# Mr-LvGJ/kubernetes-scheduler

Hardware: AMD Instinct MI355X
Metric: pod-node pair evals/sec (filter+score+select) at 100k×100k; bit-exact picks (higher is better)
Workload: dtype u32+f32+f64

## Files before the change

### kubernetes-scheduler_amd/csrc/yoda_kernels.hip

```cpp
#include <hip/hip_runtime.h>
#include <stdint.h>
#include <algorithm>
#include <type_traits>
#include <cstdlib>

#include "yoda_layout.h"
#include "yoda_launch.h"
#include "yoda_modeb.h"

#if !defined(YODA_AB_KNOBS) &&                                                         \
    (defined(YODA_ABL_K1_NOGEN) || defined(YODA_ABL_K1_NOHC) || defined(YODA_ABL_K1_NOPART) || \
     defined(YODA_ABL_K1_NOBS) || defined(YODA_ABL_K1_NOBM))
#error "YODA_ABL_* ablations give wrong results: build them with -DYODA_AB_KNOBS (tools/build_ab.sh)"
#endif

#pragma clang fp contract(off)

namespace yoda {

constexpr int64_t kI64Max = 0x7fffffffffffffffll;

static inline dim3 pod_grid(uint32_t n) { return dim3((n + kBlock - 1) / kBlock); }

template <Path P>
// ... 2272 lines not shown
          const double os = ts[k];
          const uint32_t oi = ti[k];
          ts[k] = gt ? cs : os;
          ti[k] = gt ? ci : oi;
          cs = gt ? os : cs;
          ci = gt ? oi : ci;
        }
      }
    } else {
      if (raw > best) {
        best = raw;
        idx = n;
        ties = 1;
      } else if (raw == best) {
        ++ties;
      }
      low = fmin(low, raw);
    }
  };
  if (ms.bs) {
    const BlockMask* bsw = ms.bs + (size_t)w * ms.bs_stride;
    for (uint32_t nb = n0; nb < n1; nb += kWave) {
      if (!blk_listed(ms.blk, ms.blk_stride, w, nb >> 6)) continue;
      const BlockMask bk = bsw[nb >> 6];
      uint64_t bits = bk.nz;
      while (bits) {
        const uint32_t j = (uint32_t)__builtin_ctzll(bits);
        bits &= bits - 1;
        const uint32_t n = nb + j;
        const uint64_t mj = ((bk.full >> j) & 1ull) ? live_mask : bmw[n];
        if ((mj >> lane) & 1ull) visit(n);
      }
    }
  } else {
    for (uint32_t g = n0; g < n1; g += 8) {
      const Group<uint64_t, 8> mk = load_group<uint64_t, 8>(
          reinterpret_cast<const unsigned char*>(bmw + g));
      if ((mk.v[0] | mk.v[1] | mk.v[2] | mk.v[3] | mk.v[4] | mk.v[5] | mk.v[6] | mk.v[7]) == 0)
        continue;
#pragma unroll
      for (int j = 0; j < 8; ++j) {
        const uint32_t n = g + (uint32_t)j;
        if (mk.v[j] == 0 || n >= n1) continue;
        if ((mk.v[j] >> lane) & 1ull) visit(n);
      }
    }
  }
  if (!live) return;
  if constexpr (OUT == OUT_TOPK) {
#pragma unroll
    for (int k = 0; k < TK; ++k) {
      const size_t o = ((size_t)chunk * TK + k) * n_pods + p;
      tk_s[o] = ts[k];
      tk_i[o] = ti[k];
    }
  } else {
    const size_t o = (size_t)chunk * n_pods + p;
    pbest[o] = best;
    pidx[o] = idx;
    pties[o] = ties;
    plow[o] = low;
  }
}

#ifndef YODA_K2_WAVES
#define YODA_K2_WAVES 5
#endif
template <int K, bool STATS, int TKO = 0, bool RK = false, bool MIX = true, bool Q32 = true>
__global__ __launch_bounds__(kBlock) __attribute__((amdgpu_waves_per_eu(K <= 8 ? (TKO == 0 ? YODA_K2_WAVES : (TKO <= 8 ? 4 : 3)) : 1))) void k2_block_n32(
    const unsigned char* __restrict__ nodes, const unsigned char* __restrict__ sum2,
    uint32_t n_nodes, uint32_t chunk_nodes, ScoreArgs args, uint32_t n_pods,
    const uint64_t* __restrict__ bm, uint32_t bm_stride, const BlockMask* __restrict__ bs,
    uint32_t bs_stride, const uint64_t* __restrict__ blk,
    uint32_t blk_stride, double* __restrict__ pbest,
    uint32_t* __restrict__ pidx, uint32_t* __restrict__ pties, double* __restrict__ plow,
    unsigned long long* __restrict__ stats, uint64_t* __restrict__ tk_keys, uint32_t ib) {
  constexpr uint32_t S2 = k2sum_stride(K), NS = n32_stride(K), MS = mix_stride(K);
  constexpr bool TOPK = TKO > 0;
  constexpr int TL = TOPK ? TKO : 1;
  constexpr uint32_t PSW = K + 2;
  constexpr uint32_t TAB = kWave * PSW;
  constexpr uint32_t kSets = 4, REC = 16;
  constexpr uint32_t TT = (TOPK && !RK) ? (TKO > 8 ? 3u : 2u) : 1u;
  constexpr uint32_t RECS = TAB, RCPS = TAB + kWave * REC, IDW = RCPS + 16 * (kSets + 1),
                     XTAB = IDW + kWave, LDSW = XTAB + (TT - 1) * TAB;
  auto row_base = [&](uint32_t q) -> uint32_t { return q == 0 ? 0u : XTAB + (q - 1u) * TAB; };
  __shared__ __attribute__((aligned(16))) uint32_t lds_all[kBlock / kWave][LDSW];
  const uint32_t lane = lane_id();
  uint32_t* lds = lds_all[threadIdx.x >> 6];
  const Tile tl = tile();
  const uint32_t pbk = args.pb_order ? args.pb_order[tl.pb] : tl.pb;
  const uint32_t p = pbk * kBlock + threadIdx.x;
  const uint32_t chunk = tl.chunk;
  const uint32_t n0 = chunk * chunk_nodes;
  const uint32_t n1 = min(n0 + chunk_nodes, n_nodes);
  const bool live = p < n_pods;
  const uint64_t live_mask = ballot(live);
  if (live_mask == 0) return;
  const bool trace = STATS && (stats[15] & 0xffull) == 1ull;
  const uint64_t t_start = STATS ? wall_clock64() : 0ull;
  const uint64_t* bmw = bm + (size_t)uniform_u32(p >> 6) * bm_stride;
  const BlockMask* bsw = bs ? bs + (size_t)uniform_u32(p >> 6) * bs_stride : nullptr;
  using RS = std::conditional_t<Q32, float, double>;
  ScorerN32<RS> sc;
  if (live) sc.load(args, p, n_pods);
  static_assert((kKbLevels & (kKbLevels - 1u)) == 0u && kKbLevels <= kWave, "one level per lane");
  uint32_t lev = 0u;
  if (args.levels != nullptr) lev = args.levels[lane & (kKbLevels - 1u)];
  const bool act = live && (args.cnt == nullptr || args.cnt[p] != 0u);
  const uint64_t act_mask = ballot(act);
  bool seed_le_g = false;
  if constexpr (!TOPK) {
    if (args.seed != nullptr && args.g.tab != nullptr) {
      bool le;
      if constexpr (Q32)
        le = sc.r_bw >= args.g.f_bw && sc.r_core >= args.g.f_core && sc.r_pow >= args.g.f_pow;
      else
        le = sc.r_bw >= args.g.r_bw && sc.r_core >= args.g.r_core && sc.r_pow >= args.g.r_pow;
      le = le && sc.r_free >= args.g.r_free && sc.r_tot >= args.g.r_tot;
      seed_le_g = (ballot(act && !le) == 0ull);
    }
  }
  auto rl_d = [&](double x, int l) {
    const uint64_t b = (uint64_t)__double_as_longlong(x);
    return __longlong_as_double((long long)((uint64_t)(uint32_t)__builtin_amdgcn_readlane(
        (int)(uint32_t)b, l) | ((uint64_t)(uint32_t)__builtin_amdgcn_readlane(
        (int)(uint32_t)(b >> 32), l) << 32)));
  };
  uint32_t set = 0, nsets = 0;
  bool has_set = false;
  uint64_t rem = act_mask;
  auto rl_s = [&](RS x, int l) -> RS {
    if constexpr (Q32) return __int_as_float(__builtin_amdgcn_readlane(__float_as_int(x), l));
    else return rl_d(x, l);
  };
  RS u_bw = 0, u_core = 0, u_pow = 0;
  double u_free = 0.0, u_tot = 0.0;
  for (; rem != 0ull && nsets < kSets; ++nsets) {
    const int l = __builtin_ctzll(rem);
    const RS b_bw = rl_s(sc.r_bw, l), b_core = rl_s(sc.r_core, l), b_pow = rl_s(sc.r_pow, l);
    const double b_free = rl_d(sc.r_free, l), b_tot = rl_d(sc.r_tot, l);
    const bool in = act && sc.r_bw == b_bw && sc.r_core == b_core && sc.r_pow == b_pow &&
                    sc.r_free == b_free && sc.r_tot == b_tot;
    const uint64_t in_b = ballot(in) & rem;
    if ((in_b >> lane) & 1ull) {
      set = nsets;
      has_set = true;
    }
    rem &= ~in_b;
    if (nsets == 0) {
      u_bw = b_bw;
      u_core = b_core;
      u_pow = b_pow;
      u_free = b_free;
      u_tot = b_tot;
    }
    if (lane == (uint32_t)l) {
      RS* r = reinterpret_cast<RS*>(lds + RCPS + 16 * nsets);
      r[0] = b_bw;
      r[1] = b_core;
      r[2] = b_pow;
      double* d = reinterpret_cast<double*>(lds + RCPS + 16 * nsets + 8);
      d[0] = b_free;
      d[1] = b_tot;
    }
  }
  const bool uni_max = nsets <= 1u && rem == 0ull;
  const bool rec_ok = rem == 0ull;
  RS g_bw, g_core, g_pow;
  if constexpr (Q32) {
    g_bw = args.g.f_bw;
    g_core = args.g.f_core;
    g_pow = args.g.f_pow;
  } else {
    g_bw = args.g.r_bw;
    g_core = args.g.r_core;
    g_pow = args.g.r_pow;
  }
  const bool use_g = uni_max && args.g.tab != nullptr && u_bw == g_bw && u_core == g_core &&
                     u_pow == g_pow && u_free == args.g.r_free && u_tot == args.g.r_tot;
  const uint32_t m_max = wave_max_u32(act ? sc.m : 0u), m_min = wave_min_u32(act ? sc.m : ~0u);
  const uint32_t c_max = wave_max_u32(act ? sc.c : 0u), c_min = wave_min_u32(act ? sc.c : ~0u);
  const bool dec = args.kbdec != nullptr && !use_g && act_mask != 0ull;
  const bool prune = args.kbub != nullptr && (use_g || dec);
  if (dec) {
    RS d_bw = act ? sc.r_bw : (RS)0, d_core = act ? sc.r_core : (RS)0, d_pow = act ? sc.r_pow : (RS)0;
    double d_free = act ? sc.r_free : 0.0, d_tot = act ? sc.r_tot : 0.0;
    if constexpr (Q32) {
      d_bw = wave_allreduce(d_bw, OpMaxF32{});
      d_core = wave_allreduce(d_core, OpMaxF32{});
      d_pow = wave_allreduce(d_pow, OpMaxF32{});
    } else {
      d_bw = wave_allreduce(d_bw, OpMaxF64{});
      d_core = wave_allreduce(d_core, OpMaxF64{});
      d_pow = wave_allreduce(d_pow, OpMaxF64{});
    }
    d_free = wave_allreduce(d_free, OpMaxF64{});
    d_tot = wave_allreduce(d_tot, OpMaxF64{});
    if (lane == 0) {
      RS* r = reinterpret_cast<RS*>(lds + RCPS + 16 * kSets);
      r[0] = d_bw;
      r[1] = d_core;
      r[2] = d_pow;
      double* d = reinterpret_cast<double*>(lds + RCPS + 16 * kSets + 8);
      d[0] = d_free;
      d[1] = d_tot;
    }
  }
  constexpr uint32_t KBST = kbub_stride(K);
  double thr = -1.0;
  if (prune && !TOPK && args.seed != nullptr) {
    const uint64_t sv = args.seed[uniform_u32(p >> 6)];
    if (sv != 0ull && (use_g || seed_le_g)) thr = (double)sv;
  }
  uint32_t lvw = kbub_lvl(K), l_lo = 0;
  if (prune && args.levels != nullptr) {
    l_lo = kb_level_lo(ballot(lev <= m_min), kKbLevels);
    lvw = kbub_lvl(K) + 2u * l_lo;
  }
  uint64_t thrk = 0ull;

  double ubest = -1.0;
  uint32_t uidx = 0xffffffffu, uties = 0;
  uint64_t rbest = 0;
  uint32_t ridx = 0xffffffffu, rties = 0;
  auto to_u = [](double x) {
    return (uint64_t)__double_as_longlong(x + 4503599627370496.0) - 0x4330000000000000ull;
  };
  uint32_t npart = 0;
  uint64_t pl[TL], ul[TL];
#pragma unroll
  for (int k = 0; k < TL; ++k) pl[k] = ul[k] = 0ull;
  const uint32_t imax = TOPK ? (1u << ib) - 1u : 0u;
  auto pl_insert = [&](uint64_t x) {
#pragma unroll
    for (int k = 0; k < TL; ++k) {
      const uint64_t o = pl[k];
      const bool gt = x > o;
      pl[k] = gt ? x : o;
      x = gt ? o : x;
    }
  };
  bool worked = false;
  auto block_ub = [&](uint32_t b) -> double {
    if (dec) {
      constexpr uint32_t DS = kbdec_stride();
      const uint32_t* D = args.kbdec;
      if (args.levels == nullptr) return HUGE_VAL;
      const uint32_t ok = D[sum_index(b, kDecOk, DS)];
      const uint32_t wbw = D[sum_index(b, kDecBw, DS)], wck = D[sum_index(b, kDecCk, DS)];
      const uint32_t wco = D[sum_index(b, kDecCo, DS)], wpw = D[sum_index(b, kDecPw, DS)];
      const uint32_t dl = kbdec_level(l_lo);
      const uint32_t wq = D[sum_index(b, kDecQl + dl, DS)];
      uint32_t w2[6];
      const uint32_t wsrc[3] = {kDecStat, kbdec_fl(dl), kbdec_tl(dl)};
#pragma unroll
      for (int i = 0; i < 3; ++i) {
        w2[2 * i] = D[sum_index(b, wsrc[i], DS)];
        w2[2 * i + 1] = D[sum_index(b, wsrc[i] + 1u, DS)];
      }
      __builtin_amdgcn_sched_group_barrier(0x0020, 12, 0);
      auto d64 = [&](int i) {
        return __longlong_as_double((long long)((uint64_t)w2[2 * i] | ((uint64_t)w2[2 * i + 1] << 32)));
      };
      const RS* r = reinterpret_cast<const RS*>(lds + RCPS + 16 * kSets);
      const double* rd = reinterpret_cast<const double*>(lds + RCPS + 16 * kSets + 8);
      const uint32_t sh = card_shared_terms(wbw, wck, wco, wpw, r[0], r[1], r[2]);
      const double q = (double)wq;
      const double ub = d64(0) + q * (double)sh + 3.0 * rd[0] * d64(1) + rd[1] * d64(2) + 1.0;
      return ok == 0u ? HUGE_VAL : ub;
    }
    const uint32_t* U = args.kbub;
    return __longlong_as_double((long long)((uint64_t)U[sum_index(b, lvw, KBST)] |
                                            ((uint64_t)U[sum_index(b, lvw + 1u, KBST)] << 32)));
  };
  auto pruned = [&](double ub) -> bool {
    if constexpr (TOPK) {
      if (!(ub < 4503599627370496.0)) return false;
      return ((((uint64_t)ub) << ib) | (uint64_t)imax) <= thrk;
    } else {
      return ub < thr;
    }
  };
  auto block = [&](uint32_t nb) {
    worked = false;
    const uint32_t n = nb + lane;
    const bool valid0 = n < n1;
    const uint32_t nid = (args.ids && valid0) ? args.ids[n] : n;
    if (args.ids) lds[IDW + lane] = nid;
    const bool valid = n < n1;
    BlockMask bk{0ull, 0ull};
    if (bsw) bk = bsw[nb >> 6];
    const uint32_t* s = reinterpret_cast<const uint32_t*>(sum2) + sum_index(nb, 0, S2) + lane;
    const uint4 h0 = make_uint4(s[64 * kS2Static], s[64 * (kS2Static + 1)], s[64 * kS2Clock],
                                s[64 * kS2Meta]);
    uint4 h1 = make_uint4(0u, 0u, 0u, 0u);
    if (MIX || !use_g)
      h1 = make_uint4(s[64 * kS2Bw], s[64 * kS2Core], s[64 * kS2Power], s[64 * kS2MinClk]);
    Group<uint32_t, K> fs, ts;
#pragma unroll
    for (int t = 0; t < K; ++t) fs.v[t] = s[64 * (kS2Fs + t)];
    if (use_g) {
      const uint32_t* gs = args.g.tab + sum_index(nb, 0, gtab_stride(K)) + lane;
#pragma unroll
      for (int t = 0; t < K; ++t) ts.v[t] = gs[64 * t];
    } else {
#pragma unroll
      for (int t = 0; t < K; ++t) ts.v[t] = s[64 * (kS2Fs + K + t)];
    }
    uint64_t mask, feas_b;
    if (bsw) {
      mask = ((bk.full >> lane) & 1ull) ? live_mask : 0ull;
      if (((bk.nz & ~bk.full) >> lane) & 1ull) mask = bmw[n];
      feas_b = bk.nz;
    } else {
      mask = valid ? bmw[n] : 0ull;
      feas_b = ballot(mask != 0ull);
    }
    if (feas_b == 0) return;
    worked = true;
    if (STATS && !trace && lane == 0) atomicAdd(stats + 14, 1ull);
    uint64_t fast_b = 0, u_b = 0, rec_b = 0;
    uint32_t ck = h0.z;
    bool fast = mask != 0ull && (!MIX || (h0.w & kSumUni4) != 0u);
    uint64_t ub_key = ~0ull;
    {
      const uint32_t meta = h0.w, bw = h1.x, core = h1.y, pw = h1.z;
      const uint32_t cnt = (meta >> 8) & 0xffu;
      uint32_t nq_lo = 0, nq_hi = 0;
#pragma unroll
      for (int t = 0; t < K; ++t) {
        nq_lo += (uint32_t)(fs.v[t] >= m_max);
        nq_hi += (uint32_t)(fs.v[t] >= m_min);
      }
      nq_lo = min(nq_lo, cnt);
      nq_hi = min(nq_hi, cnt);
      const uint32_t range = nq_hi - nq_lo;
      uint32_t* rec = lds + RECS + lane * REC;
      if constexpr (K >= 4) {
#pragma unroll
        for (int t = 0; t < K; t += 4)
          *reinterpret_cast<uint4*>(rec + t) =
              make_uint4(fs.v[t], fs.v[t + 1], fs.v[t + 2], fs.v[t + 3]);
      } else {
#pragma unroll
        for (int t = 0; t < K; ++t) rec[t] = fs.v[t];
      }
      const uint32_t thr = nq_lo < (uint32_t)K ? rec[nq_lo] : 0u;
      const uint32_t thr1 = range > 1u && nq_lo + 1u < (uint32_t)K ? rec[nq_lo + 1u] : 0u;
      const uint32_t thr2 = range > 2u && nq_lo + 2u < (uint32_t)K ? rec[nq_lo + 2u] : 0u;
      const double stat_d =
          __longlong_as_double((long long)((uint64_t)h0.x | ((uint64_t)h0.y << 32)));
      const uint64_t stat_u = (uint64_t)__double_as_longlong(stat_d + 4503599627370496.0) -
                              0x4330000000000000ull;
      if (uni_max) {
        uint32_t sel = 0, sel_hi = 0;
        lds[lane * PSW + 0] = 0u;
        if (use_g) {
#pragma unroll
          for (int t = 0; t < K; ++t) {
            const uint32_t b = ts.v[t];
            lds[lane * PSW + t + 1] = b;
            if constexpr (TOPK) sel_hi = (uint32_t)(t + 1) == nq_hi ? b : sel_hi;
          }
          sel = lds[lane * PSW + nq_lo];
        } else {
          const uint32_t shared = card_shared_terms(bw, ck, core, pw, u_bw, u_core, u_pow);
          auto row = [&](auto rk) {
            uint32_t acc = 0;
#pragma unroll
            for (int t = 0; t < K; ++t) {
              acc += mem_term<decltype(rk)::value>(fs.v[t], ts.v[t], u_free, u_tot, args.mt);
              const uint32_t b = (uint32_t)(t + 1) * shared + acc;
              lds[lane * PSW + t + 1] = b;
              if constexpr (TOPK) sel_hi = (uint32_t)(t + 1) == nq_hi ? b : sel_hi;
            }
          };
          row(std::integral_constant<bool, RK>{});
          sel = lds[lane * PSW + nq_lo];
        }
        const bool mixn = MIX && mask != 0ull && (meta & kSumUni4) == 0u;
        if (ballot(mixn) != 0ull) {
          if (mixn) {
            bool ok = use_g && h1.w >= c_max;
            if (!ok) {
              const uint32_t* mxw = args.mix + sum_index(nb, 0, MS) + lane;
              bool cu = true;
              sel = 0u;
              sel_hi = 0u;
              auto row = [&](auto rk) {
                uint32_t acc = 0;
#pragma unroll
                for (int t = 0; t < K; ++t) {
                  const uint32_t cj = mxw[64 * mix_word(kMixCk, t, K)];
                  const uint32_t to = use_g ? s[64 * (kS2Fs + K + t)] : ts.v[t];
                  cu = cu && ((cj >= c_max) || (cj < c_min));
                  const uint32_t term =
                      card_shared_terms(mxw[64 * mix_word(kMixBw, t, K)], cj,
                                        mxw[64 * mix_word(kMixCo, t, K)],
                                        mxw[64 * mix_word(kMixPw, t, K)], u_bw, u_core, u_pow) +
                      mem_term<decltype(rk)::value>(fs.v[t], to, u_free, u_tot, args.mt);
                  acc += cj >= c_max ? term : 0u;
                  lds[lane * PSW + t + 1] = acc;
                  sel = (uint32_t)(t + 1) == nq_lo ? acc : sel;
                  if constexpr (TOPK) sel_hi = (uint32_t)(t + 1) == nq_hi ? acc : sel_hi;
                }
              };
              row(std::integral_constant<bool, RK>{});
              ok = cu;
            }
            fast = ok;
            ck = ~0u;
          }
        }
        if constexpr (TOPK) {
          const uint64_t ub = stat_u + (ck >= c_min ? sel_hi : 0u);
          if (fast) ub_key = (ub << ib) | (uint64_t)(imax - n);
        }
        const double stat = stat_d;
        const bool q_all = ck >= c_max, q_none = ck < c_min;
        const bool is_u = fast && mask == act_mask && nq_lo == nq_hi && (q_all || q_none);
        u_b = ballot(is_u);
        if constexpr (TOPK) {
          const uint32_t basic = q_all ? sel : 0u;
          const uint64_t key =
              is_u ? ((stat_u + basic) << ib) | (uint64_t)(imax - n) : 0ull;
          bool cand = key > ul[TL - 1];
          while (ballot(cand) != 0ull) {
            uint64_t x = wave_max_u64(cand ? key : 0ull);
            cand = cand && key != x;
#pragma unroll
            for (int k = 0; k < TL; ++k) {
              const uint64_t o = ul[k];
              const bool gt = x > o;
              ul[k] = gt ? x : o;
              x = gt ? o : x;
            }
            cand = cand && key > ul[TL - 1];
          }
        } else {
          const uint32_t basic = q_all ? sel : 0u;
          const double raw = (double)basic + stat;
          const bool gt = is_u && raw > ubest, eq = is_u && raw == ubest;
          uidx = gt ? nid : (eq ? min(uidx, nid) : uidx);
          uties = gt ? 1u : uties + (eq ? 1u : 0u);
          ubest = gt ? raw : ubest;
        }
        const bool is_rec = fast && range <= 3u && !is_u;
        rec_b = ballot(is_rec);
        if (is_rec) {
          const uint32_t* row = lds + lane * PSW;
          const uint32_t q1 = nq_lo + min(range, 1u), q2 = nq_lo + min(range, 2u);
          const uint32_t q3 = nq_lo + min(range, 3u);
          *reinterpret_cast<uint4*>(rec) = make_uint4(ck, (uint32_t)mask, (uint32_t)(mask >> 32),
                                                      thr);
          *reinterpret_cast<uint4*>(rec + 4) = make_uint4((uint32_t)stat_u,
                                                          (uint32_t)(stat_u >> 32), thr1, thr2);
          *reinterpret_cast<uint4*>(rec + 8) =
              make_uint4(sel, row[q1], row[q2], row[q3]);
        }
      } else {
        const bool is_rec = !RK && rec_ok && fast && range <= 1u;
        rec_b = ballot(is_rec);
        if (!RK && (rec_b != 0ull || (TT > 1u && ballot(fast && !is_rec) != 0ull))) {
          if (is_rec) {
            *reinterpret_cast<uint4*>(rec) = make_uint4(ck, (uint32_t)mask,
                                                        (uint32_t)(mask >> 32), thr);
            *reinterpret_cast<uint4*>(rec + 4) = make_uint4((uint32_t)stat_u,
                                                            (uint32_t)(stat_u >> 32), 0u, 0u);
          }
          for (uint32_t q = 0; q < nsets; ++q) {
            const RS* r = reinterpret_cast<const RS*>(lds + RCPS + 16 * q);
            const double* d = reinterpret_cast<const double*>(lds + RCPS + 16 * q + 8);
            const double v_free = d[0], v_tot = d[1];
            const uint32_t shared = card_shared_terms(bw, ck, core, pw, r[0], r[1], r[2]);
            uint32_t sel = 0, sel_hi = 0;
            uint32_t* trow = lds + row_base(q < TT ? q : 0u) + lane * PSW;
            const bool wrow = TT > 1u && q < TT;
            if (wrow) trow[0] = 0u;
            auto row = [&](auto rk) {
              uint32_t acc = 0;
#pragma unroll
              for (int t = 0; t < K; ++t) {
                acc += mem_term<decltype(rk)::value>(fs.v[t], ts.v[t], v_free, v_tot, args.mt);
                sel = (uint32_t)(t + 1) == nq_lo ? acc : sel;
                sel_hi = (uint32_t)(t + 1) == nq_hi ? acc : sel_hi;
                if (wrow) trow[t + 1] = (uint32_t)(t + 1) * shared + acc;
              }
            };
            row(std::integral_constant<bool, RK>{});
            if (is_rec)
              *reinterpret_cast<uint2*>(rec + 8 + 2 * q) =
                  make_uint2(nq_lo * shared + sel, nq_hi * shared + sel_hi);
          }
        }
      }
    }
    fast_b = ballot(fast);
    uint64_t part_b = feas_b & ~u_b;
    if constexpr (TOPK) {
      const uint64_t thr = wave_min_u64(act ? pl[TL - 1] : ~0ull);
      const uint64_t keep_b = ballot(ub_key > thr);
      part_b &= keep_b;
      rec_b &= keep_b;
    }
    if (STATS && !trace && lane == 0) {
      atomicAdd(stats + 2, (unsigned long long)__builtin_popcountll(u_b));
      atomicAdd(stats + 3, (unsigned long long)__builtin_popcountll(part_b & fast_b));
      atomicAdd(stats + 4, (unsigned long long)__builtin_popcountll(part_b & ~fast_b));
      atomicAdd(stats + 7, (unsigned long long)__builtin_popcountll(rec_b));
      if (!uni_max) atomicAdd(stats + 8, (unsigned long long)__builtin_popcountll(part_b));
    }
    if (STATS) npart += (uint32_t)__builtin_popcountll(part_b);
    uint64_t rb = rec_b;
    part_b &= ~rec_b;
    auto take_r = [&](bool f, uint64_t raw, uint32_t nn) {
      if constexpr (TOPK) {
        const uint64_t key = f ? (raw << ib) | (uint64_t)(imax - nn) : 0ull;
        if (key > pl[TL - 1]) pl_insert(key);
        return;
      }
      const bool gt = f & (raw > rbest), eq = f & (raw == rbest);
      ridx = gt ? nn : (eq ? min(ridx, nn) : ridx);
      rties = gt ? 1u : rties + (eq ? 1u : 0u);
      rbest = gt ? raw : rbest;
    };
    while (rb) {
#ifndef YODA_K2_R
#define YODA_K2_R 2
#endif
      constexpr int R = YODA_K2_R;
      uint32_t jj[R];
      bool vv[R];
#pragma unroll
      for (int k = 0; k < R; ++k) {
        vv[k] = rb != 0ull;
        jj[k] = vv[k] ? (uint32_t)__builtin_ctzll(rb) : 0u;
        rb &= rb - 1;
      }
      uint4 ra[R], rs[R], rp[R];
#pragma unroll
      for (int k = 0; k < R; ++k) {
        const uint32_t* r = lds + RECS + jj[k] * REC;
        ra[k] = *reinterpret_cast<const uint4*>(r);
        rs[k] = *reinterpret_cast<const uint4*>(r + 4);
        if (uni_max) {
          rp[k] = *reinterpret_cast<const uint4*>(r + 8);
        } else {
          const uint2 pr = *reinterpret_cast<const uint2*>(r + 8 + 2 * set);
          rp[k] = make_uint4(pr.x, pr.y, pr.y, pr.y);
        }
      }
#pragma unroll
      for (int k = 0; k < R; ++k) {
        const bool c0 = sc.m <= ra[k].w, c1 = sc.m <= rs[k].z, c2 = sc.m <= rs[k].w;
        const uint32_t bsel = c2 ? rp[k].w : (c1 ? rp[k].z : (c0 ? rp[k].y : rp[k].x));
        const uint32_t basic = ra[k].x >= sc.c ? bsel : 0u;
        const uint64_t raw = ((uint64_t)rs[k].x | ((uint64_t)rs[k].y << 32)) + basic;
        const uint32_t mw = lane < 32u ? ra[k].y : ra[k].z;
        take_r(vv[k] && ((mw >> (lane & 31u)) & 1u) != 0u, raw,
               args.ids ? lds[IDW + jj[k]] : nb + jj[k]);
      }
    }
    while (part_b) {
      const int j = __builtin_ctzll(part_b);
      part_b &= part_b - 1;
      const uint32_t nn =
          args.ids ? (uint32_t)__builtin_amdgcn_readlane((int)nid, j) : nb + (uint32_t)j;
      const uint64_t mj =
          ((uint64_t)(uint32_t)__builtin_amdgcn_readlane((int)(uint32_t)(mask >> 32), j) << 32) |
          (uint32_t)__builtin_amdgcn_readlane((int)(uint32_t)mask, j);
      if constexpr (TOPK) {
        const uint64_t ubj =
            ((uint64_t)(uint32_t)__builtin_amdgcn_readlane((int)(uint32_t)(ub_key >> 32), j)
             << 32) |
            (uint32_t)__builtin_amdgcn_readlane((int)(uint32_t)ub_key, j);
        if (ballot(((mj >> lane) & 1ull) != 0ull && ubj > pl[TL - 1]) == 0ull) continue;
      }
      double raw;
      if (!MIX || ((fast_b >> j) & 1ull)) {
        const uint32_t cnt = ((uint32_t)__builtin_amdgcn_readlane((int)h0.w, j) >> 8) & 0xffu;
        uint32_t nq = 0;
#pragma unroll
        for (int t = 0; t < K; ++t)
          nq += (uint32_t)((uint32_t)__builtin_amdgcn_readlane((int)fs.v[t], j) >= sc.m);
        nq = min(nq, cnt);
        const uint32_t ckj = (uint32_t)__builtin_amdgcn_readlane((int)ck, j);
        const uint64_t sb = (uint64_t)(uint32_t)__builtin_amdgcn_readlane((int)h0.x, j) |
                            ((uint64_t)(uint32_t)__builtin_amdgcn_readlane((int)h0.y, j) << 32);
        uint32_t basic;
        if (uni_max) {
          const uint32_t* tab = lds + (uint32_t)j * PSW;
          basic = ckj >= sc.c ? tab[nq] : 0u;
        } else if (TT > 1u &&
                   ballot(((mj >> lane) & 1ull) != 0ull && !(has_set && set < TT)) == 0ull) {
          const uint32_t* tab = lds + row_base(set) + (uint32_t)j * PSW;
          basic = ckj >= sc.c ? tab[nq] : 0u;
        } else {
          const auto& own = sc;
          const uint32_t shared = card_shared_terms(
              (uint32_t)__builtin_amdgcn_readlane((int)h1.x, j), ckj,
              (uint32_t)__builtin_amdgcn_readlane((int)h1.y, j),
              (uint32_t)__builtin_amdgcn_readlane((int)h1.z, j), own.r_bw, own.r_core, own.r_pow);
          uint32_t mem = 0;
          auto terms = [&](auto rk) {
#pragma unroll
            for (int t = 0; t < K; ++t) {
              const uint32_t f = (uint32_t)__builtin_amdgcn_readlane((int)fs.v[t], j);
              const uint32_t to = (uint32_t)__builtin_amdgcn_readlane((int)ts.v[t], j);
              const uint32_t term =
                  mem_term<decltype(rk)::value>(f, to, own.r_free, own.r_tot, args.mt);
              mem += (uint32_t)t < nq ? term : 0u;
            }
          };
          terms(std::integral_constant<bool, RK>{});
          basic = ckj >= sc.c ? nq * shared + mem : 0u;
        }
        raw = (double)basic + __longlong_as_double((long long)sb);
      } else {
        raw = sc.template raw<K>(nodes + (size_t)nn * NS);
      }
      take_r(((mj >> lane) & 1ull) != 0ull, to_u(raw), nn);
    }
  };
  unsigned long long gpub = 0ull;
  auto refresh_thr_g = [&](unsigned long long g) {
    const double wu = wave_allreduce(ubest, OpMaxF64{});
    double lb = act ? fmax(rties > 0u ? (double)rbest : -1.0, wu) : HUGE_VAL;
    if (args.gbest != nullptr && act) {
      const unsigned long long mine = lb >= 0.0 ? (unsigned long long)lb + 1ull : 0ull;
      if (mine > g && mine > gpub) {
        atomicMax(args.gbest + p, mine);
        gpub = mine;
      }
      lb = fmax(lb, (double)g - 1.0);
    }
    lb = wave_allreduce(lb, OpMinF64{});
    thr = fmax(thr, __longlong_as_double(
                        (long long)uniform_u64((uint64_t)__double_as_longlong(lb))));
  };
  auto load_gbest = [&]() -> unsigned long long {
    return (args.gbest != nullptr && act) ? args.gbest[p] : 0ull;
  };
  auto refresh_thr = [&]() { refresh_thr_g(load_gbest()); };
  auto refresh_thrk_g = [&](unsigned long long g) {
    uint64_t kth = act ? (pl[TL - 1] > ul[TL - 1] ? pl[TL - 1] : ul[TL - 1]) : ~0ull;
    if (args.gbest != nullptr && act) {
      if (kth > g) atomicMax(args.gbest + p, (unsigned long long)kth);
      kth = kth > g ? kth : g;
    }
    thrk = wave_min_u64(kth);
  };
  auto refresh_thrk = [&]() { refresh_thrk_g(load_gbest()); };
  const uint64_t t_setup = STATS ? wall_clock64() : 0ull;
  if (blk) {
    const uint64_t* bw = blk + (size_t)uniform_u32(p >> 6) * blk_stride;
    const uint32_t b0 = n0 >> 6, b1 = (n1 + 63) >> 6;
    const bool hot_first = prune && args.hot != nullptr;
    const uint64_t* hw = hot_first ? args.hot : bw;
    for (uint32_t wb = b0; wb < b1; wb += kWave) {
      const uint64_t bits_w = window_bits(bw, blk_stride, wb, b1);
      const uint64_t hot_w = window_bits(hw, blk_stride, wb, b1);
      const unsigned long long g_w = prune ? load_gbest() : 0ull;
      double ub_l = 0.0;
      if (prune) {
        ub_l = block_ub(min(wb + lane, b1 - 1u));
        if (args.gbest != nullptr) {
          if constexpr (TOPK) refresh_thrk_g(g_w); else refresh_thr_g(g_w);
        }
      }
      uint64_t todo = bits_w;
      auto drop_pruned = [&]() {
        const uint64_t cand = ballot(!pruned(ub_l));
        if (STATS && !trace && lane == 0 && (todo & ~cand) != 0ull)
          atomicAdd(stats + 13, (unsigned long long)__builtin_popcountll(todo & ~cand));
        todo &= cand;
      };
      if (prune) drop_pruned();
      while (todo != 0ull) {
        const uint64_t first = (todo & hot_w) != 0ull ? (todo & hot_w) : todo;
        const uint32_t j = (uint32_t)__builtin_ctzll(first);
        todo &= ~(1ull << j);
        block((wb + j) << 6);
        if (prune && worked) {
          if constexpr (TOPK) refresh_thrk(); else refresh_thr();
          drop_pruned();
        }
      }
    }
  } else {
    for (uint32_t nb = n0; nb < n1; nb += kWave) block(nb);
  }
  const uint64_t t_pass = STATS ? wall_clock64() : 0ull;
  if (STATS && !trace && lane == 0) {
    atomicAdd(stats + 5, uni_max ? 1ull : 0ull);
    atomicAdd(stats + 6, 1ull);
    atomicMax(stats + 9, (unsigned long long)npart);
  }
  const size_t slot2 = (size_t)(p >> 6) * gridDim.y + chunk;
  if (trace && lane == 0 && slot2 < (size_t)(stats[15] >> 8)) {
    {
      unsigned long long* tr = stats + 16 + 4 * slot2;
      tr[0] = t_start;
      tr[1] = wall_clock64();
      tr[2] = npart;
      tr[3] = (uni_max ? 1ull : 0ull) | (use_g ? 2ull : 0ull) | (dec ? 4ull : 0ull) |
              ((unsigned long long)nsets << 4) |
              ((unsigned long long)min((unsigned long long)(t_setup - t_start), 0xffffffull) << 16) |
              ((unsigned long long)min((unsigned long long)(t_pass - t_start), 0xffffffull) << 40);
    }
  }
  if constexpr (TOPK) {
#pragma unroll
    for (int k = 0; k < TL; ++k) {
      const uint64_t x = act ? ul[k] : 0ull;
      const bool take = x > pl[TL - 1];
      if (ballot(take) == 0ull) break;
      if (take) pl_insert(x);
    }
    if (!live) return;
    uint64_t* o = tk_keys + ((size_t)chunk * n_pods + p) * TL;
#pragma unroll
    for (int k = 0; k < TL; k += 2)
      *reinterpret_cast<ulonglong2*>(o + k) = make_ulonglong2(pl[k], pl[k + 1]);
    return;
  }
  double wb = ubest;
#pragma unroll
  for (int o = kWave / 2; o > 0; o >>= 1) wb = fmax(wb, __shfl_xor(wb, o, kWave));
  const bool top = ubest == wb && uties > 0;
  uint32_t wi = top ? uidx : 0xffffffffu, wt = top ? uties : 0u;
#pragma unroll
  for (int o = kWave / 2; o > 0; o >>= 1) {
    wi = min(wi, (uint32_t)__shfl_xor((int)wi, o, kWave));
    wt += (uint32_t)__shfl_xor((int)wt, o, kWave);
  }
  double best = rties > 0 ? (double)rbest : -1.0;
  uint32_t idx = ridx, ties = rties;
  if (act && wt > 0) {
    if (wb > best) {
      best = wb;
      idx = wi;
      ties = wt;
    } else if (wb == best) {
      idx = min(idx, wi);
      ties += wt;
    }
  }
  if (args.cmask != nullptr) {
    bool useful = live && act && best >= 0.0;
    if (useful && args.gbest != nullptr)
      useful = (unsigned long long)best + 1ull >= args.gbest[p];
    if (ballot(useful) == 0ull) return;
    if (lane == 0) atomicOr(args.cmask + (p >> 6), 1ull << chunk);
  }
  if (!live) return;
  const size_t o = (size_t)chunk * n_pods + p;
  pbest[o] = best;
  pidx[o] = idx;
  pties[o] = ties;
}

template <int TK>
__global__ __launch_bounds__(kBlock) void k_topk_merge(const double* __restrict__ tk_s,
                                                       const uint32_t* __restrict__ tk_i,
                                                       uint32_t C, uint32_t n_pods,
                                                       uint32_t node_offset,
                                                       double* __restrict__ out_s,
                                                       uint32_t* __restrict__ out_i) {
  const uint32_t p = blockIdx.x * kBlock + threadIdx.x;
  if (p >= n_pods) return;
  double ts[TK];
  uint32_t ti[TK];
#pragma unroll
  for (int k = 0; k < TK; ++k) {
    ts[k] = -1.0;
    ti[k] = 0xffffffffu;
  }
  for (uint32_t c = 0; c < C; ++c) {
    for (int e = 0; e < TK; ++e) {
      const size_t o = ((size_t)c * TK + e) * n_pods + p;
      double cs = tk_s[o];
      uint32_t ci = tk_i[o];
      if (!(cs > ts[TK - 1])) break;
#pragma unroll
      for (int k = 0; k < TK; ++k) {
        const bool gt = cs > ts[k] || (cs == ts[k] && ci < ti[k]);
        const double os = ts[k];
        const uint32_t oi = ti[k];
        ts[k] = gt ? cs : os;
// ... 973 lines not shown
      ++sn.n;
    }
  }
  if constexpr (!ELIG) sn.first = sn.n ? n0 + threadIdx.x : 0xffffffffu;
  uint32_t mc, mi;
  disk_settle(s, sn, mc, mi);
  const uint32_t L = wave_max_u32(mc ? s.lev : 0u);
  uint32_t cnt = s.lev == L ? mc : 0u;
  uint32_t idx = (s.lev == L && mc) ? mi : 0xffffffffu;
#pragma unroll
  for (int o = kWave / 2; o > 0; o >>= 1) {
    cnt += (uint32_t)__shfl_xor((int)cnt, o, kWave);
    idx = min(idx, (uint32_t)__shfl_xor((int)idx, o, kWave));
  }
  const uint32_t w = threadIdx.x / kWave;
  if (lane_id() == 0) {
    red[0][w] = L;
    red[1][w] = cnt;
    red[2][w] = idx;
  }
  __syncthreads();
  if (threadIdx.x != 0) return;
  DiskBest b;
  disk_best_init(b);
  for (int i = 0; i < kBlock / kWave; ++i) disk_merge_any(b, red[0][i], red[1][i], red[2][i]);
  plc[(size_t)chunk * n_cls + c] = b.cnt ? disk_pack((uint32_t)b.lev, b.cnt) : 0u;
  pidx[(size_t)chunk * n_cls + c] = b.idx;
}

__global__ __launch_bounds__(kBlock) void k_reduce2b(const uint32_t* __restrict__ plc,
                                                     const uint32_t* __restrict__ pidx,
                                                     uint32_t C, uint32_t n_cls,
                                                     const uint32_t* __restrict__ cls,
                                                     uint32_t n_pods, uint32_t node_offset,
                                                     int64_t* __restrict__ best_out,
                                                     uint32_t* __restrict__ idx_out,
                                                     uint32_t* __restrict__ ties_out,
                                                     int64_t* __restrict__ low_out) {
  const uint32_t p = blockIdx.x * kBlock + threadIdx.x;
  if (p >= n_pods) return;
  const uint32_t c = cls[p];
  DiskBest b;
  disk_best_init(b);
  for (uint32_t k = 0; k < C; ++k)
    disk_merge_chunk(b, plc[(size_t)k * n_cls + c], &pidx[(size_t)k * n_cls + c]);
  best_out[p] = b.lev;
  idx_out[p] = b.idx == 0xffffffffu ? b.idx : b.idx + node_offset;
  ties_out[p] = b.cnt;
  low_out[p] = 0;
}

struct Reduce2Out {
  int64_t best, low;
  uint32_t idx, ties;
};
__device__ __forceinline__ Reduce2Out reduce2_pod(
    const double* __restrict__ pbest_f, const int64_t* __restrict__ pbest_i,
    const uint32_t* __restrict__ pidx, const uint32_t* __restrict__ pties,
    const double* __restrict__ plow_f, const int64_t* __restrict__ plow_i, uint32_t C,
    uint32_t n_pods, int is_f64, uint32_t node_offset, uint32_t p,
    const unsigned long long* __restrict__ cmask) {
  int64_t best = -1, low = kI64Max;
  uint32_t idx = 0xffffffffu, ties = 0;
  uint64_t bits = cmask != nullptr ? cmask[p >> 6] : 0ull;
  const uint32_t CN = cmask != nullptr ? (uint32_t)__builtin_popcountll(bits) : C;
#pragma unroll 4
  for (uint32_t k = 0; k < CN; ++k) {
    uint32_t c = k;
    if (cmask != nullptr) {
      c = (uint32_t)__builtin_ctzll(bits);
      bits &= bits - 1ull;
    }
    const size_t o = (size_t)c * n_pods + p;
    int64_t b, l;
    if (is_f64) {
      const double bf = pbest_f[o], lf = plow_f ? plow_f[o] : 1.0e300;
      b = bf < 0.0 ? -1 : (int64_t)bf;
      l = lf > 9.0e18 ? kI64Max : (int64_t)lf;
    } else {
      b = pbest_i[o];
      l = plow_i[o];
    }
    const uint32_t ix = pidx[o], tt = pties[o];
    const bool v = b >= 0, gt = v && b > best, eq = v && b == best;
    idx = gt ? ix : (eq ? min(idx, ix) : idx);
    ties = gt ? tt : (eq ? ties + tt : ties);
    best = gt ? b : best;
    low = (v && l < low) ? l : low;
  }
  Reduce2Out r;
  r.best = best;
  r.idx = idx == 0xffffffffu ? idx : idx + node_offset;
  r.ties = ties;
  r.low = (is_f64 && !plow_f) ? best : low;
  return r;
}

__global__ __launch_bounds__(kBlock) void k_reduce2(const double* __restrict__ pbest_f,
                                                    const int64_t* __restrict__ pbest_i,
                                                    const uint32_t* __restrict__ pidx,
                                                    const uint32_t* __restrict__ pties,
                                                    const double* __restrict__ plow_f,
                                                    const int64_t* __restrict__ plow_i,
                                                    uint32_t C, uint32_t n_pods, int is_f64,
                                                    uint32_t node_offset,
                                                    int64_t* __restrict__ best_out,
                                                    uint32_t* __restrict__ idx_out,
                                                    uint32_t* __restrict__ ties_out,
                                                    int64_t* __restrict__ low_out,
                                                    const unsigned long long* __restrict__ cmask = nullptr) {
  const uint32_t p = blockIdx.x * kBlock + threadIdx.x;
  if (p >= n_pods) return;
  const Reduce2Out r = reduce2_pod(pbest_f, pbest_i, pidx, pties, plow_f, plow_i, C, n_pods,
                                   is_f64, node_offset, p, cmask);
  best_out[p] = r.best;
  idx_out[p] = r.idx;
  ties_out[p] = r.ties;
  low_out[p] = r.low;
}

__global__ __launch_bounds__(kWave) void k_reduce2_wave(const double* __restrict__ pbest_f,
                                                         const int64_t* __restrict__ pbest_i,
                                                         const uint32_t* __restrict__ pidx,
                                                         const uint32_t* __restrict__ pties,
                                                         const double* __restrict__ plow_f,
                                                         const int64_t* __restrict__ plow_i,
                                                         uint32_t C, uint32_t n_pods, int is_f64,
                                                         uint32_t node_offset,
                                                         int64_t* __restrict__ best_out,
                                                         uint32_t* __restrict__ idx_out,
                                                         uint32_t* __restrict__ ties_out,
                                                         int64_t* __restrict__ low_out) {
  const uint32_t p = blockIdx.x, lane = threadIdx.x;
  int64_t best = -1, low = kI64Max;
  uint32_t idx = 0xffffffffu, ties = 0;
  for (uint32_t c = lane; c < C; c += kWave) {
    const size_t o = (size_t)c * n_pods + p;
    int64_t b, l;
    if (is_f64) {
      const double bf = pbest_f[o], lf = plow_f ? plow_f[o] : 1.0e300;
      b = bf < 0.0 ? -1 : (int64_t)bf;
      l = lf > 9.0e18 ? kI64Max : (int64_t)lf;
    } else {
      b = pbest_i[o];
      l = plow_i[o];
    }
    if (b < 0) continue;
    if (b > best) {
      best = b;
      idx = pidx[o];
      ties = pties[o];
    } else if (b == best) {
      ties += pties[o];
      idx = min(idx, pidx[o]);
    }
    low = l < low ? l : low;
  }
  for (int o = kWave / 2; o > 0; o >>= 1) {
    const int64_t ob = __shfl_xor(best, o, kWave);
    const uint32_t oi = __shfl_xor(idx, o, kWave);
    const uint32_t ot = __shfl_xor(ties, o, kWave);
    const int64_t ol = __shfl_xor(low, o, kWave);
    if (ob > best) {
      best = ob;
      idx = oi;
      ties = ot;
    } else if (ob == best && ob >= 0) {
      ties += ot;
      idx = min(idx, oi);
    }
    low = ol < low ? ol : low;
// ... 2483 lines not shown
```

### kubernetes-scheduler_amd/csrc/yoda_layout.h

```cpp
#pragma once
#include <stdint.h>

namespace yoda {

constexpr int kBlock = 256;
constexpr int kWave = 64;
constexpr uint32_t kChunkAlign = 64;

enum class Path : int { N32 = 0, F64 = 1, U64 = 2 };
constexpr uint64_t kFastFieldMax = 1ull << 44;
constexpr uint64_t kFastScoreMax = 1ull << 52;
constexpr uint64_t kN32FieldMax = 0xFFFFFFFEull;
constexpr uint64_t kF32SmallMax = 55738;

struct alignas(16) NodeHdrF {
  double static_score;
  uint64_t card_number;
  uint32_t healthy_mask;
  uint32_t zero_total;
  uint32_t real_mask;
  uint32_t flags;
};
constexpr uint32_t kNodeUniform4 = 1u;
constexpr uint32_t kNodeUniformTotal = 2u;
// ... 30 lines not shown
};
constexpr uint32_t kSumUni4 = 1u, kSumUniTotal = 2u, kSumZeroTotal = 4u;
constexpr uint32_t kSumAbsent = 8u;
__host__ __device__ constexpr uint32_t k1sum_stride(int k) {
  return (48u + 4u * (uint32_t)k + 15u) & ~15u;
}

enum K2SumWord { kS2Static = 0, kS2Clock = 2, kS2Meta = 3, kS2Bw = 4, kS2Core = 5, kS2Power = 6,
                 kS2MinClk = 7, kS2Fs = 8 };
__host__ __device__ constexpr uint32_t k2sum_stride(int k) { return 32u + 8u * (uint32_t)k; }

enum BlockSumWord {
  kBsCnMin = 0, kBsCnMax = 1, kBsFlags = 2, kBsCkMin = 3, kBsCkMax = 4, kBsHckMin = 5,
  kBsHckMax = 6, kBsNhMin = 7, kBsNhMax = 8, kBsMrfMin = 9, kBsMrfMax = 10, kBsNReal = 11,
  kBsNzt = 12, kBsMx = 13, kBsWc = 19, kBsWl = 25, kBsSat = 31, kBsHc = 32, kBsT = 36
};
constexpr uint32_t kBsOneModel = 1u, kBsUni4 = 2u, kBsHcTab = 4u, kBsAbsent = 8u;
__host__ __device__ constexpr uint32_t bsum_stride(int k) { return 4u * (kBsT + 2u * (uint32_t)k); }

constexpr uint32_t kKbLevels = 64;
__host__ __device__ constexpr uint32_t kbub_lvl(int) { return 0u; }
__host__ __device__ constexpr uint32_t kbub_stride(int k) {
  return (4u * (kbub_lvl(k) + 2u * kKbLevels) + 15u) & ~15u;
}
__host__ __device__ inline uint64_t kb_low_bits(uint32_t n) {
  return n >= 64u ? ~0ull : (1ull << n) - 1ull;
}
__host__ __device__ inline uint32_t kb_level_lo(uint64_t le_mask, uint32_t n_levels) {
  return (uint32_t)__builtin_popcountll(le_mask & kb_low_bits(n_levels) & ~1ull);
}
__host__ __device__ inline uint32_t kb_level_hi(uint64_t lt_mask, uint32_t n_levels) {
  return (uint32_t)__builtin_popcountll(lt_mask & kb_low_bits(n_levels - 1u));
}

enum KbDecWord { kDecOk = 0, kDecBw = 1, kDecCk = 2, kDecCo = 3, kDecPw = 4, kDecStat = 5, kDecQl = 7 };
constexpr uint32_t kKbDecLevels = kKbLevels / 2u;
__host__ __device__ constexpr uint32_t kbdec_level(uint32_t l) { return l >> 1; }
__host__ __device__ constexpr uint32_t kbdec_fl(uint32_t d) { return kDecQl + kKbDecLevels + 2u * d; }
__host__ __device__ constexpr uint32_t kbdec_tl(uint32_t d) { return kDecQl + 3u * kKbDecLevels + 2u * d; }
__host__ __device__ constexpr uint32_t kbdec_stride() {
  return (4u * (kDecQl + 5u * kKbDecLevels) + 15u) & ~15u;
}

enum MixWord { kMixCk = 0, kMixBw = 1, kMixCo = 2, kMixPw = 3 };
__host__ __device__ constexpr uint32_t mix_word(int field, int j, int k) {
  return (uint32_t)(field * k + j);
}
__host__ __device__ constexpr uint32_t mix_hm(int k) { return 4u * (uint32_t)k; }
__host__ __device__ constexpr uint32_t mix_stride(int k) { return 4u * (4u * (uint32_t)k + 1u); }

enum K1MixWord { kX1Chg = 0, kX1Ch = 1, kX1Pm = 5 };
__host__ __device__ constexpr uint32_t x1_pm(int q1, int f) { return kX1Pm + 3u * (uint32_t)q1 + (uint32_t)f; }
__host__ __device__ constexpr uint32_t x1_cd(int t, int f, int k) {
  return kX1Pm + 3u * (uint32_t)k + 2u * (uint32_t)t + (uint32_t)f;
}
__host__ __device__ constexpr uint32_t x1_stride(int k) { return 4u * (kX1Pm + 5u * (uint32_t)k); }
constexpr uint32_t kX1ChgMany = 1u << 31;

__host__ __device__ constexpr size_t sum_index(uint32_t n, uint32_t w, uint32_t stride) {
  return ((size_t)(n >> 6) * (stride / 4u) + w) * 64u + (n & 63u);
}
__host__ __device__ constexpr size_t sum_words(uint32_t n_nodes, uint32_t stride) {
  return (size_t)((n_nodes + 63u) >> 6) * 64u * (stride / 4u);
}

__host__ __device__ constexpr uint32_t bm_row(uint32_t n_nodes) { return (n_nodes + 63u) & ~63u; }
struct alignas(16) BlockMask {
  uint64_t nz, full;
};
__host__ __device__ constexpr uint32_t bs_row(uint32_t n_nodes) { return (n_nodes + 63u) / 64u; }
__host__ __device__ constexpr uint32_t blk_row(uint32_t n_nodes) {
  return ((n_nodes + 63u) / 64u + 63u) / 64u;
}
__host__ __device__ inline uint64_t window_bits(const uint64_t* words, uint32_t row_words,
                                                uint32_t wb, uint32_t b1) {
  const uint32_t wi = wb >> 6, sh = wb & 63u;
  const bool two = sh != 0u && wi + 1u < row_words && ((wi + 1u) << 6) < b1;
  const uint64_t lo = words[wi], hi = words[two ? wi + 1u : wi];
  uint64_t bits = lo >> sh;
  if (two) bits |= hi << (64u - sh);
  const uint32_t n = b1 - wb;
  if (n < 64u) bits &= (1ull << n) - 1ull;
  return bits;
}

struct alignas(16) K1WaveRec {
  uint64_t num_min, num_max;
  uint32_t mpm_min, mpm_max;
  uint32_t m_min, m_max, c_min, c_max;
  uint32_t cpc_max, nc_min, nc_max;
  uint32_t nm_min, nm_max;
  uint32_t flags;
};
static_assert(sizeof(K1WaveRec) == 64, "K1WaveRec layout");
constexpr uint32_t kK1RecAnyPm = 1u, kK1RecAllPm = 2u, kK1RecAnyPc = 4u, kK1RecAllPc = 8u,
                   kK1RecCUni = 16u;

struct PermCopy {
  const uint32_t* inv = nullptr;
  unsigned char* sum = nullptr;
  unsigned char* sum2 = nullptr;
  uint32_t* mix = nullptr;
  uint32_t* x1 = nullptr;
  uint32_t* bsum = nullptr;
  uint32_t* bsum_p = nullptr;
  uint32_t bsum_words = 0;
};

struct alignas(16) NodeRecB {
  double v, u;
};

struct DiskLevels {
  double t[12];
};
constexpr uint32_t kDiskCountBits = 28;
struct DiskPlan {
  uint32_t chunk, C;
  bool node_lanes;
};

struct OnePod {
  uint64_t number;
  uint32_t need_mem, need_clk;
  uint32_t m32, c32;
  double mf, cf;
};
struct alignas(16) OneOut {
  uint64_t maxima[6];
  uint32_t nf, nz, first, pad;
  double rcp[5];
  double best, low;
  uint32_t idx, ties;
};

struct alignas(8) ShardRec {
  int64_t best;
  uint32_t idx, ties;
  int64_t low;
};
static_assert(sizeof(ShardRec) == 24, "ShardRec layout");
constexpr int kMaxLocalShards = 16;
struct PtrList {
  const void* p[kMaxLocalShards];
};

struct GTab {
  const uint32_t* tab;
  double r_bw, r_core, r_pow, r_free, r_tot;
  float f_bw, f_core, f_pow;
};
__host__ __device__ constexpr uint32_t gtab_stride(int k) { return 4u * (uint32_t)k; }

struct MemTab {
  const double* vf = nullptr;
  const double* vt = nullptr;
  uint32_t nf = 0;
};

struct PodParams {
  double* m_f;
  double* c_f;
  uint64_t* m_u;
  uint64_t* c_u;
  uint32_t* m_32;
  uint32_t* c_32;
// ... 183 lines not shown
```

Before: 26110 billion.

## Widen record path to cover score ranges up to three for K=8 in k2

```diff
diff --git a/kubernetes-scheduler_amd/csrc/yoda_kernels.hip b/kubernetes-scheduler_amd/csrc/yoda_kernels.hip
--- a/kubernetes-scheduler_amd/csrc/yoda_kernels.hip
+++ b/kubernetes-scheduler_amd/csrc/yoda_kernels.hip
@@ -2378,6 +2378,8 @@
   constexpr uint32_t TAB = kWave * PSW;
   constexpr uint32_t kSets = 4, REC = 16;
   constexpr uint32_t TT = (TOPK && !RK) ? (TKO > 8 ? 3u : 2u) : 1u;
+  constexpr bool WIDE = !TOPK && !RK && K == 8 && Q32 && (!MIX || STATS);
+  static_assert(!WIDE || PSW % 2u == 0u, "a table row's word pairs are read as 8-byte words");
   constexpr uint32_t RECS = TAB, RCPS = TAB + kWave * REC, IDW = RCPS + 16 * (kSets + 1),
                      XTAB = IDW + kWave, LDSW = XTAB + (TT - 1) * TAB;
   auto row_base = [&](uint32_t q) -> uint32_t { return q == 0 ? 0u : XTAB + (q - 1u) * TAB; };
@@ -2524,6 +2526,9 @@
     return (uint64_t)__double_as_longlong(x + 4503599627370496.0) - 0x4330000000000000ull;
   };
   uint32_t npart = 0;
+  uint32_t nwork = 0;
+  uint32_t nrec = 0;
+  uint32_t nwide = 0;
   uint64_t pl[TL], ul[TL];
 #pragma unroll
   for (int k = 0; k < TL; ++k) pl[k] = ul[k] = 0ull;
@@ -2615,6 +2620,7 @@
     }
     if (feas_b == 0) return;
     worked = true;
+    if (STATS) ++nwork;
     if (STATS && !trace && lane == 0) atomicAdd(stats + 14, 1ull);
     uint64_t fast_b = 0, u_b = 0, rec_b = 0;
     uint32_t ck = h0.z;
@@ -2756,9 +2762,48 @@
               make_uint4(sel, row[q1], row[q2], row[q3]);
         }
       } else {
-        const bool is_rec = !RK && rec_ok && fast && range <= 1u;
+        const bool is_rec = !RK && rec_ok && fast && range <= (WIDE ? 3u : 1u);
         rec_b = ballot(is_rec);
-        if (!RK && (rec_b != 0ull || (TT > 1u && ballot(fast && !is_rec) != 0ull))) {
+        if constexpr (WIDE) {
+          if (rec_b != 0ull) {
+            if (STATS) nwide += (uint32_t)__builtin_popcountll(ballot(is_rec && range > 1u));
+            if (is_rec) {
+              *reinterpret_cast<uint4*>(rec) = make_uint4(ck, (uint32_t)mask,
+                                                          (uint32_t)(mask >> 32), thr);
+              *reinterpret_cast<uint4*>(rec + 4) = make_uint4((uint32_t)stat_u,
+                                                              (uint32_t)(stat_u >> 32), thr1, thr2);
+            }
+            const uint32_t npass = ballot(is_rec && range > 1u) != 0ull ? 2u : 1u;
+#pragma nounroll
+            for (uint32_t pass = 0; pass < npass; ++pass) {
+              const uint32_t qa = nq_lo + min(range, 2u * pass), qb = nq_lo + min(range, 2u * pass + 1u);
+#pragma nounroll
+              for (uint32_t q = 0; q < nsets; ++q) {
+                const RS* r = reinterpret_cast<const RS*>(lds + RCPS + 16 * q);
+                const double* d = reinterpret_cast<const double*>(lds + RCPS + 16 * q + 8);
+                const double v_free = d[0], v_tot = d[1];
+                const uint32_t shared = card_shared_terms(bw, ck, core, pw, r[0], r[1], r[2]);
+                uint32_t acc = 0, sa = 0, sb = 0;
+#pragma unroll
+                for (int t = 0; t < K; ++t) {
+                  acc += mem_term<false>(fs.v[t], ts.v[t], v_free, v_tot, args.mt);
+                  sa = (uint32_t)(t + 1) == qa ? acc : sa;
+                  sb = (uint32_t)(t + 1) == qb ? acc : sb;
+                }
+                if (is_rec) {
+                  uint32_t* v = q < 2u ? rec + 8 + 4 * q : lds + lane * PSW + 4 * (q - 2u);
+                  const uint2 ab = make_uint2(qa * shared + sa, qb * shared + sb);
+                  if (pass == 0u) {
+                    *reinterpret_cast<uint2*>(v) = ab;
+                    *reinterpret_cast<uint2*>(v + 2) = make_uint2(ab.y, ab.y);
+                  } else {
+                    *reinterpret_cast<uint2*>(v + 2) = ab;
+                  }
+                }
+              }
+            }
+          }
+        } else if (!RK && (rec_b != 0ull || (TT > 1u && ballot(fast && !is_rec) != 0ull))) {
           if (is_rec) {
             *reinterpret_cast<uint4*>(rec) = make_uint4(ck, (uint32_t)mask,
                                                         (uint32_t)(mask >> 32), thr);
@@ -2808,6 +2853,7 @@
       if (!uni_max) atomicAdd(stats + 8, (unsigned long long)__builtin_popcountll(part_b));
     }
     if (STATS) npart += (uint32_t)__builtin_popcountll(part_b);
+    if (STATS) nrec += (uint32_t)__builtin_popcountll(rec_b);
     uint64_t rb = rec_b;
     part_b &= ~rec_b;
     auto take_r = [&](bool f, uint64_t raw, uint32_t nn) {
@@ -2842,6 +2888,11 @@
         rs[k] = *reinterpret_cast<const uint4*>(r + 4);
         if (uni_max) {
           rp[k] = *reinterpret_cast<const uint4*>(r + 8);
+        } else if constexpr (WIDE) {
+          const uint32_t* v = set < 2u ? r + 8 + 4 * set : lds + jj[k] * PSW + 4 * (set - 2u);
+          const uint2 lo = *reinterpret_cast<const uint2*>(v);
+          const uint2 hi = *reinterpret_cast<const uint2*>(v + 2);
+          rp[k] = make_uint4(lo.x, lo.y, hi.x, hi.y);
         } else {
           const uint2 pr = *reinterpret_cast<const uint2*>(r + 8 + 2 * set);
           rp[k] = make_uint4(pr.x, pr.y, pr.y, pr.y);
@@ -2974,8 +3025,7 @@
       };
       if (prune) drop_pruned();
       while (todo != 0ull) {
-        const uint64_t first = (todo & hot_w) != 0ull ? (todo & hot_w) : todo;
-        const uint32_t j = (uint32_t)__builtin_ctzll(first);
+        const uint32_t j = k2_claim_pick(todo, hot_w);
         todo &= ~(1ull << j);
         block((wb + j) << 6);
         if (prune && worked) {
@@ -2999,9 +3049,10 @@
       unsigned long long* tr = stats + 16 + 4 * slot2;
       tr[0] = t_start;
       tr[1] = wall_clock64();
-      tr[2] = npart;
+      tr[2] = npart | ((unsigned long long)min(nwork, 0xffffu) << 32) |
+              ((unsigned long long)min(nrec, 0xffffu) << 48);
       tr[3] = (uni_max ? 1ull : 0ull) | (use_g ? 2ull : 0ull) | (dec ? 4ull : 0ull) |
-              ((unsigned long long)nsets << 4) |
+              ((unsigned long long)nsets << 4) | ((unsigned long long)min(nwide, 0xffu) << 8) |
               ((unsigned long long)min((unsigned long long)(t_setup - t_start), 0xffffffull) << 16) |
               ((unsigned long long)min((unsigned long long)(t_pass - t_start), 0xffffffull) << 40);
     }
@@ -4141,11 +4192,8 @@
       l = plow_i[o];
     }
     const uint32_t ix = pidx[o], tt = pties[o];
-    const bool v = b >= 0, gt = v && b > best, eq = v && b == best;
-    idx = gt ? ix : (eq ? min(idx, ix) : idx);
-    ties = gt ? tt : (eq ? ties + tt : ties);
-    best = gt ? b : best;
-    low = (v && l < low) ? l : low;
+    argmax_fold(best, idx, ties, b, ix, tt);
+    low = (b >= 0 && l < low) ? l : low;
   }
   Reduce2Out r;
   r.best = best;
diff --git a/kubernetes-scheduler_amd/csrc/yoda_layout.h b/kubernetes-scheduler_amd/csrc/yoda_layout.h
--- a/kubernetes-scheduler_amd/csrc/yoda_layout.h
+++ b/kubernetes-scheduler_amd/csrc/yoda_layout.h
@@ -136,6 +136,27 @@
   const uint32_t n = b1 - wb;
   if (n < 64u) bits &= (1ull << n) - 1ull;
   return bits;
+}
+
+struct ArgmaxState {
+  int64_t best = -1;
+  uint32_t idx = 0xffffffffu, ties = 0u;
+};
+__host__ __device__ inline void argmax_fold(int64_t& best, uint32_t& idx, uint32_t& ties,
+                                            int64_t b, uint32_t ix, uint32_t tt) {
+  const bool v = b >= 0, gt = v && b > best, eq = v && b == best;
+  const uint32_t lo = ix < idx ? ix : idx;
+  idx = gt ? ix : (eq ? lo : idx);
+  ties = gt ? tt : (eq ? ties + tt : ties);
+  best = gt ? b : best;
+}
+__host__ __device__ inline void argmax_fold(ArgmaxState& a, const ArgmaxState& b) {
+  argmax_fold(a.best, a.idx, a.ties, b.best, b.idx, b.ties);
+}
+
+__host__ __device__ inline uint32_t k2_claim_pick(uint64_t todo, uint64_t hot) {
+  const uint64_t first = (todo & hot) != 0ull ? (todo & hot) : todo;
+  return (uint32_t)__builtin_ctzll(first);
 }
 
 struct alignas(16) K1WaveRec {
```

Result: faster. 27520 billion, median of 6 (+5.4%).
